# ml4ai/mliis

Measured on AMD Instinct MI355X. Metric: inner-loop images/sec (EfficientLab-6-3, 224x224, 5-shot), higher is better.
Workload: dtype f32 (the long-K decoder convs and their filter gradients with every operand split exactly into three bf16 terms on the matrix cores, 6 term products, f32 accumulate: fp32-equivalent products; everything else the fp32 instruction)

## Files before the change

### mliis_amd/csrc/conv_x3.hip

```cpp
#include "conv_gemm_kernels.hpp"

namespace mliis {

constexpr int kX3BM = 256;
#ifndef X3_PF
#define X3_PF 1
#endif
constexpr int kX3PF = X3_PF;

__global__ __launch_bounds__(128) void x3_pack_k(const float* __restrict__ theta, char* __restrict__ images, const long long* __restrict__ desc,
                                                  int ndesc) {
  x3_pack_block(theta, images, desc, ndesc, blockIdx.x, threadIdx.x);
}

struct X3Params {
  ConvGemmParams g;
  const char* image;
  int ncol16;
#ifdef X3_CLK
  unsigned long long* dbg;
#endif
};

template <int NT>
struct X3Sm {
  static constexpr int BN = 16 * NT;
  static constexpr int B_BYTES = NT * kX3Block;
  static constexpr int STAGES = 2;
  static constexpr int BYTES = STAGES * B_BYTES + 64;
};

template <int NT>
__device__ __forceinline__ void conv_x3_tile(const X3Params& q, char* __restrict__ sm, unsigned bx, int by, int it0, int it1,
                                             float* __restrict__ pdst) {
  constexpr int BN = 16 * NT;
  constexpr int B_BYTES = X3Sm<NT>::B_BYTES;
  constexpr int NB = (NT * 192 + 511) / 512;
  const ConvGemmParams& p = q.g;
  const int t = threadIdx.x, lane = t & 63;
  const int wave = __builtin_amdgcn_readfirstlane(t >> 6);
  const int l15 = lane & 15, g = lane >> 4;
  const long long M = (long long)p.Nimg * p.H * p.W;
  const long long m0 = (long long)bx * kX3BM;
  const int n0 = by * BN;
  const __amdgpu_buffer_rsrc_t rA = __builtin_amdgcn_make_buffer_rsrc((void*)p.A, 0, kBufRecords, 0x00020000);
  const __amdgpu_buffer_rsrc_t rB = __builtin_amdgcn_make_buffer_rsrc((void*)q.image, 0, kBufRecords, 0x00020000);

  const int wrow = wave * 32;
  unsigned a_row[2], a_taps[2];
#pragma unroll
  for (int rb = 0; rb < 2; ++rb) {
    const long long m = m0 + wrow + rb * 16 + l15;
    a_taps[rb] = 0;
    a_row[rb] = 0;
    if (m < M) {
      a_row[rb] = (unsigned)(m * p.lda * 4);
      if (p.ntaps > 1) {
        const int HWp = p.H * p.W;
        const int n = (int)(m / HWp);
        const int rem = (int)(m - (long long)n * HWp);
        const int h = rem / p.W, w_ = rem - h * p.W;
#pragma unroll
        for (int tp = 0; tp < 9; ++tp) {
          const int dh = (tp / 3 - 1) * p.dil * p.sign, dw = (tp % 3 - 1) * p.dil * p.sign;
          if ((unsigned)(h + dh) < (unsigned)p.H && (unsigned)(w_ + dw) < (unsigned)p.W) a_taps[rb] |= 1u << tp;
        }
      } else {
        a_taps[rb] = 1u;
      }
    }
  }
  int l_tap[2], l_c[2];
#pragma unroll
  for (int qd = 0; qd < 2; ++qd) {
    const int k0 = it0 * 32 + qd * 16 + g * 4;
    l_tap[qd] = k0 / p.C;
    l_c[qd] = k0 - l_tap[qd] * p.C;
  }
  int s_aleft = it1 - it0, s_bleft = it1 - it0;
  int ncol_here = q.ncol16 - by * NT;
  if (ncol_here > NT) ncol_here = NT;
  const unsigned b_lim = (unsigned)ncol_here * 192u;
  const unsigned b_step = (unsigned)q.ncol16 * kX3Block;
  unsigned b_voff[NB];
#pragma unroll
  for (int i = 0; i < NB; ++i) b_voff[i] = ((unsigned)t + 512u * i < b_lim) ? (unsigned)(by * NT) * kX3Block + ((unsigned)t + 512u * i) * 16u : kOob;
  unsigned s_boff = (unsigned)it0 * b_step;

  float4 ra[2][2];
  float4 ra2[2][2];
  u32x4 rbv[NB];
  const int tap_scale = p.dil * p.sign;
  auto load_a_into = [&](float4 (&ra)[2][2]) {
    const int adv = s_aleft > 1 ? 1 : 0;
    s_aleft -= adv;
#pragma unroll
    for (int qd = 0; qd < 2; ++qd) {
      const int tap = l_tap[qd];
      const int th = p.ntaps > 1 ? (tap * 11) >> 5 : 1, tw = p.ntaps > 1 ? tap - 3 * th : 1;
      const int dh = (th - 1) * tap_scale, dw = (tw - 1) * tap_scale;
      const unsigned koff = (unsigned)(((dh * p.W + dw) * p.lda + l_c[qd]) * 4);
      const unsigned tapbit = tap < p.ntaps ? 1u << tap : 0u;
#pragma unroll
      for (int rb = 0; rb < 2; ++rb) ra[rb][qd] = buf_ld4(rA, (a_taps[rb] & tapbit) != 0 ? a_row[rb] + koff : kOob);
      const int c_next = l_c[qd] + 32;
      const int wrap = c_next >= p.C ? 1 : 0;
      l_c[qd] = adv ? (wrap ? c_next - p.C : c_next) : l_c[qd];
      l_tap[qd] += adv & wrap;
    }
  };
  auto load_b_into = [&](u32x4 (&rbv)[NB]) {
#pragma unroll
    for (int i = 0; i < NB; ++i) {
      rbv[i] = __builtin_amdgcn_raw_buffer_load_b128(rB, (int)b_voff[i], (int)s_boff, 0);
    }
    const int adv = s_bleft > 1 ? 1 : 0;
    s_bleft -= adv;
    s_boff += adv ? b_step : 0u;
  };
  auto store_b_from = [&](char* buf, const u32x4 (&rbv)[NB]) {
#pragma unroll
    for (int i = 0; i < NB; ++i) {
      const int idx = t + 512 * i;
      char* d = (512 * (i + 1) <= NT * 192 || idx < NT * 192) ? buf + idx * 16 : sm + X3Sm<NT>::STAGES * B_BYTES + (t & 3) * 16;
      *reinterpret_cast<u32x4*>(d) = rbv[i];
    }
  };
  auto load_b = [&]() { load_b_into(rbv); };
  auto store_b = [&](char* buf) { store_b_from(buf, rbv); };
  bf16x8 a3[3][2], a3n[3][2];
  auto split_into = [&](const float4 (&ra)[2][2], bf16x8 (&a3)[3][2]) {
#pragma unroll
    for (int rb = 0; rb < 2; ++rb) {
      uint2 h0, m0_, l0, h1, m1, l1;
      split3(ra[rb][0], h0, m0_, l0);
      split3(ra[rb][1], h1, m1, l1);
      a3[0][rb] = __builtin_bit_cast(bf16x8, (u32x4){h0.x, h0.y, h1.x, h1.y});
      a3[1][rb] = __builtin_bit_cast(bf16x8, (u32x4){m0_.x, m0_.y, m1.x, m1.y});
      a3[2][rb] = __builtin_bit_cast(bf16x8, (u32x4){l0.x, l0.y, l1.x, l1.y});
    }
  };
  f32x4 acc[2][NT];
#pragma unroll
  for (int rb = 0; rb < 2; ++rb)
#pragma unroll
    for (int j = 0; j < NT; ++j) acc[rb][j] = (f32x4){0.f, 0.f, 0.f, 0.f};
  auto compute_split = [&](const char* buf, const float4 (&rs)[2][2]) {
    const char* pb = buf + g * 256 + l15 * 16;
    constexpr int PF = kX3PF;
    bf16x8 b3[PF + 1][3];
    uint2 sh[2][2], sm_[2][2], sl[2][2];
#pragma unroll
    for (int d = 0; d < PF; ++d)
      if (d < NT) {
#pragma unroll
        for (int pl = 0; pl < 3; ++pl) b3[d][pl] = *reinterpret_cast<const bf16x8*>(pb + d * kX3Block + pl * 1024);
      }
#pragma unroll
    for (int jn = 0; jn < NT; ++jn) {
#if defined(X3_ABL) && (X3_ABL & 2)
      if (jn + PF < NT && jn + PF < 2) {
#else
      if (jn + PF < NT) {
#endif
#pragma unroll
        for (int pl = 0; pl < 3; ++pl) b3[(jn + PF) % (PF + 1)][pl] = *reinterpret_cast<const bf16x8*>(pb + (jn + PF) * kX3Block + pl * 1024);
      }
#define X3_MM(PA, PB)                                                                                                           \
  acc[0][jn] = __builtin_amdgcn_mfma_f32_16x16x32_bf16(a3[PA][0], b3[jn % (PF + 1)][PB], acc[0][jn], 0, 0, 0);                \
  acc[1][jn] = __builtin_amdgcn_mfma_f32_16x16x32_bf16(a3[PA][1], b3[jn % (PF + 1)][PB], acc[1][jn], 0, 0, 0);
#if defined(X3_ABL) && (X3_ABL & 1)
      X3_MM(0, 0)
#else
      X3_MM(2, 0) X3_MM(0, 2) X3_MM(1, 1) X3_MM(1, 0) X3_MM(0, 1) X3_MM(0, 0)
#endif
#undef X3_MM
#pragma unroll
      for (int k = 0; k < 4; ++k)
        if ((k * NT) / 4 == jn) {
          uint2& h = sh[k >> 1][k & 1];
          uint2& m = sm_[k >> 1][k & 1];
          uint2& l = sl[k >> 1][k & 1];
#ifdef X3_NOSPLIT
          h = make_uint2(__float_as_uint(rs[k >> 1][k & 1].x), __float_as_uint(rs[k >> 1][k & 1].y));
          m = make_uint2(__float_as_uint(rs[k >> 1][k & 1].z), __float_as_uint(rs[k >> 1][k & 1].w));
          l = h;
#else
          split3(rs[k >> 1][k & 1], h, m, l);
#endif
          asm volatile("" : "+v"(h.x), "+v"(h.y), "+v"(m.x), "+v"(m.y), "+v"(l.x), "+v"(l.y));
        }
      __builtin_amdgcn_sched_barrier(0);
    }
#pragma unroll
    for (int rb = 0; rb < 2; ++rb) {
      a3n[0][rb] = __builtin_bit_cast(bf16x8, (u32x4){sh[rb][0].x, sh[rb][0].y, sh[rb][1].x, sh[rb][1].y});
      a3n[1][rb] = __builtin_bit_cast(bf16x8, (u32x4){sm_[rb][0].x, sm_[rb][0].y, sm_[rb][1].x, sm_[rb][1].y});
      a3n[2][rb] = __builtin_bit_cast(bf16x8, (u32x4){sl[rb][0].x, sl[rb][0].y, sl[rb][1].x, sl[rb][1].y});
    }
  };
#ifdef X3_CLK
  const unsigned long long ck0 = __builtin_amdgcn_s_memtime(), cr0 = __builtin_amdgcn_s_memrealtime();
  unsigned long long c_comp = 0, c_skel = 0, c_bar = 0, c_t = ck0;
#define X3_TICK(acc_) do { const unsigned long long n_ = __builtin_amdgcn_s_memtime(); acc_ += n_ - c_t; c_t = n_; } while (0)
#else
#define X3_TICK(acc_) do { } while (0)
#endif
  const int nper = it1 - it0;
  load_a_into(ra);
  load_b();
  store_b(sm);
  load_b();
  split_into(ra, a3);
  load_a_into(ra);
  load_a_into(ra2);
  lds_barrier();
  auto chunk = [&](char* cur, char* nxt, float4 (&rs)[2][2]) {
    compute_split(cur, rs);
    X3_TICK(c_comp);
#if !(defined(X3_ABL) && (X3_ABL & 8))
    store_b(nxt);
    load_b();
#endif
#if !(defined(X3_ABL) && (X3_ABL & 4))
    load_a_into(rs);
#endif
    X3_TICK(c_skel);
    lds_barrier();
    X3_TICK(c_bar);
#pragma unroll
    for (int pl = 0; pl < 3; ++pl)
#pragma unroll
      for (int rb = 0; rb < 2; ++rb) a3[pl][rb] = a3n[pl][rb];
  };
  {
    int it = 0;
    for (; it + 2 <= nper; it += 2) {
      chunk(sm, sm + B_BYTES, ra);
      chunk(sm + B_BYTES, sm, ra2);
    }
    if (it < nper) chunk(sm, sm + B_BYTES, ra);
  }
#ifndef X3_NO_DRAIN
  asm volatile("s_waitcnt vmcnt(0)" ::: "memory");
#endif
#ifdef X3_CLK
  if (q.dbg != nullptr && lane == 0 && (wave & 3) == 0) {
    unsigned long long* d = q.dbg + ((long long)blockIdx.x * 2 + (wave >> 2)) * 8;
    if (d[0] == 0) {
      d[0] = ck0;
      d[1] = cr0;
      d[2] = __builtin_amdgcn_s_memtime();
      d[3] = __builtin_amdgcn_s_memrealtime();
      d[4] = c_comp;
      d[5] = c_skel;
      d[6] = c_bar;
      d[7] = nper;
    }
  }
#endif
#pragma unroll
  for (int rb = 0; rb < 2; ++rb)
#pragma unroll
    for (int r = 0; r < 4; ++r) {
      const int row = wrow + rb * 16 + g * 4 + r;
      if (m0 + row >= M) continue;
#pragma unroll
      for (int j = 0; j < NT; ++j)
        if (n0 + j * 16 + l15 < p.Nout) pdst[(long long)row * BN + j * 16 + l15] = acc[rb][j][r];
    }
}

template <int NT>
__global__ __launch_bounds__(512) void conv_x3_k(X3Params q, SkPlan k) {
  __shared__ __attribute__((aligned(16))) char sm[X3Sm<NT>::BYTES];
  constexpr int BN = 16 * NT;
#ifndef X3_NO_CLAIM
  asm volatile("v_mov_b32 v255, 0" ::: "v255");
#endif
#ifndef X3_NO_XCD
  const int part = (int)xcd_remap(blockIdx.x, gridDim.x);
#else
  const int part = blockIdx.x;
#endif
  int lo = part * k.ipp;
  const int total = k.rem * k.nchunks;
  int hi = lo + k.ipp;
  if (hi > total) hi = total;
#pragma unroll 1
  while (lo < hi) {
    const int rt = lo / k.nchunks, c0 = lo - rt * k.nchunks;
    int c1 = c0 + (hi - lo);
    if (c1 > k.nchunks) c1 = k.nchunks;
    const int first = (rt * k.nchunks) / k.ipp;
    float* dst = k.slab + ((long long)rt * k.smax + (part - first)) * (kX3BM * BN);
    conv_x3_tile<NT>(q, sm, rt / k.gy, rt % k.gy, c0, c1, dst);
    lo += c1 - c0;
    __syncthreads();
  }
}

constexpr int kX3Fix = 4;
template <int NT>
__global__ __launch_bounds__(1024) void x3_fixup_k(ConvGemmParams p, SkPlan k) {
  constexpr int BN = 16 * NT, QN = BN / 4;
  constexpr int QS = QN <= 32 ? 32 : 64;
  constexpr int RL = 1024 / QS;
  constexpr int RPT = kX3BM / kX3Fix / RL;
  __shared__ float4 red[2][RL][QS];
  const int t = threadIdx.x, q = t % QS, rl = t / QS;
  const int rt = blockIdx.x, sub = blockIdx.y;
  const unsigned tau = k.full + rt;
  const int bx = tau / k.gy, by = tau % k.gy;
  const long long M = (long long)p.Nimg * p.H * p.W;
  const int r0 = sub * (kX3BM / kX3Fix);
  const long long m0 = (long long)bx * kX3BM + r0;
  const int n = by * BN + q * 4;
  const bool cok = q < QN && n < p.Nout;
  const int first = (rt * k.nchunks) / k.ipp;
  int last = ((rt + 1) * k.nchunks - 1) / k.ipp;
  if (last > k.parts - 1) last = k.parts - 1;
  const int nslots = last - first + 1;
  const float* base = k.slab + ((long long)rt * k.smax * kX3BM + r0) * BN + q * 4;
  float4 s1 = f4zero(), s2 = f4zero();
  if (cok) {
    const float4 bv = p.bias != nullptr ? ld4(p.bias + n) : f4zero();
    const long long HWp = (long long)p.H * p.W;
    float4 v[RPT];
#pragma unroll
    for (int i = 0; i < RPT; ++i) v[i] = (m0 + rl + RL * i < M) ? ld4(base + (long long)(rl + RL * i) * BN) : f4zero();
    for (int z = 1; z < nslots; ++z) {
      float4 u[RPT];
#pragma unroll
      for (int i = 0; i < RPT; ++i) u[i] = (m0 + rl + RL * i < M) ? ld4(base + ((long long)z * kX3BM + rl + RL * i) * BN) : f4zero();
#pragma unroll
      for (int i = 0; i < RPT; ++i) v[i] = f4add(v[i], u[i]);
    }
#pragma unroll
    for (int i = 0; i < RPT; ++i) {
      const long long m = m0 + rl + RL * i;
      if (m >= M) continue;
      float4 o = f4add(v[i], bv);
      if (p.border_bias != nullptr) {
        const int ni = (int)(m / HWp);
        const int rem = (int)(m - (long long)ni * HWp);
        const int h = rem / p.W, w_ = rem - h * p.W;
        const int cls = (h == 0 ? 0 : (h == p.H - 1 ? 2 : 1)) * 3 + (w_ == 0 ? 0 : (w_ == p.W - 1 ? 2 : 1));
        o = f4add(o, ld4(p.border_bias + ((long long)ni * 9 + cls) * p.Nout + n));
      }
      float* dst = p.Cmat + m * p.ldc + n;
      if (p.accumulate) o = f4add(o, ld4(dst));
      st4(dst, o);
      if (p.stats_swish) o = make_float4(swish_f(o.x), swish_f(o.y), swish_f(o.z), swish_f(o.w));
      s1 = f4add(s1, o);
      s2 = f4fma(o, o, s2);
    }
  }
  if (p.stats_part == nullptr) return;
  red[0][rl][q] = s1;
  red[1][rl][q] = s2;
  __syncthreads();
  if (t < 2 * QS) {
    const int v = t / QS, qq = t % QS;
    const int nn = by * BN + qq * 4;
    if (qq < QN && nn < p.Nout) {
      float4 a = red[v][0][qq];
#pragma unroll 8
      for (int r = 1; r < RL; ++r) a = f4add(a, red[v][r][qq]);
      st4(p.stats_part + (((long long)bx * kX3Fix + sub) * 2 + v) * p.Nout + nn, a);
    }
  }
}

typedef short x3_v4s __attribute__((ext_vector_type(4)));
__device__ __forceinline__ uint2 ds_read_tr16(const char* p) {
  const x3_v4s r = __builtin_amdgcn_ds_read_tr16_b64_v4i16((x3_v4s __attribute__((address_space(3)))*)(p));
  return __builtin_bit_cast(uint2, r);
}
constexpr int kF3Rows = 32;
constexpr int kF3Plane = kF3Rows * 256;
constexpr int kF3Stage = 6 * kF3Plane;
__device__ __forceinline__ int f3_swz(int row) { return (row & 3) | (((row >> 3) & 1) << 2); }

template <int BCI>
struct F3Sm {
  static constexpr int XQ = BCI / 4;
  static constexpr int XP = BCI * 2;
  static constexpr int X_PLANE = kF3Rows * XP;
  static constexpr int STAGE = 3 * X_PLANE + 3 * kF3Plane;
};
template <int NT, int BCI>
__device__ __forceinline__ void conv_filter_x3_body(const FilterGradParams& p, char* __restrict__ sm, int bx, int by, int bz) {
  constexpr int BN = 16 * NT;
  constexpr bool WIDE = BCI == 256;
  constexpr int XQ = F3Sm<BCI>::XQ, XP = F3Sm<BCI>::XP, X_PLANE = F3Sm<BCI>::X_PLANE, STAGE = F3Sm<BCI>::STAGE;
  constexpr int X_PER_THREAD = kF3Rows * XQ / 512;
  constexpr int X_ROWS_PASS = 512 / XQ;
  constexpr int D_TOTAL = kF3Rows * (BN / 4);
  constexpr int D_PER_THREAD = (D_TOTAL + 511) / 512;
  constexpr int NT0 = WIDE ? NT : (NT + 1) / 2, NT1 = WIDE ? 0 : NT / 2;
  const int t = threadIdx.x, lane = t & 63;
  const int wave = __builtin_amdgcn_readfirstlane(t >> 6);
  const int cib = WIDE ? wave : (wave & 3), half = WIDE ? 0 : (wave >> 2);
  const int l15 = lane & 15, g = lane >> 4;
  const int M = p.Nimg * p.H * p.W;
  const bool mt = p.multitap != 0;
  const int cblocks = mt ? 1 : (p.C + BCI - 1) / BCI;
  const int tap = mt ? 0 : bx / cblocks;
  const int ci0 = mt ? 0 : (bx - tap * cblocks) * BCI;
  const int n0 = by * BN;
#ifdef F3_SAMEBZ
  const int mbeg = 0;
#else
  const int mbeg = bz * p.rows_per_split;
#endif
  int mend = mbeg + p.rows_per_split;
  if (mend > M) mend = M;
  const int HW = p.H * p.W;
  const int adv_h = kF3Rows / p.W, adv_w = kF3Rows - adv_h * p.W;
  const __amdgpu_buffer_rsrc_t rX = __builtin_amdgcn_make_buffer_rsrc((void*)p.X, 0, kBufRecords, 0x00020000);
  const __amdgpu_buffer_rsrc_t rD = __builtin_amdgcn_make_buffer_rsrc((void*)p.dY, 0, kBufRecords, 0x00020000);

  const int x_cq = t % XQ, x_r0 = t / XQ;
  int l_tap = tap, l_c = ci0 + x_cq * 4;
  if (mt) {
    l_tap = (x_cq * 4) / p.C;
    l_c = x_cq * 4 - l_tap * p.C;
  }
  const bool x_cok = mt ? l_tap < p.ntaps : l_c < p.C;
  int dh = 0, dw = 0;
  if (p.ntaps > 1) {
    dh = (l_tap / 3 - 1) * p.dil;
    dw = (l_tap % 3 - 1) * p.dil;
  }
  int x_m[X_PER_THREAD], x_h[X_PER_THREAD], x_w[X_PER_THREAD];
  unsigned x_off[X_PER_THREAD];
#pragma unroll
  for (int i = 0; i < X_PER_THREAD; ++i) {
    const int m = mbeg + x_r0 + X_ROWS_PASS * i;
    x_m[i] = m;
    const int n = m / HW;
    const int rem = m - n * HW;
    x_h[i] = rem / p.W;
    x_w[i] = rem - x_h[i] * p.W;
    x_off[i] = (unsigned)((((long long)m + (long long)dh * p.W + dw) * p.ldx + l_c) * 4);
  }
  const unsigned x_step = (unsigned)(kF3Rows * p.ldx * 4);
  int d_m[D_PER_THREAD];
  unsigned d_off[D_PER_THREAD];
  bool d_ok[D_PER_THREAD];
  int d_lds[D_PER_THREAD];
#pragma unroll
  for (int i = 0; i < D_PER_THREAD; ++i) {
    const int idx = t + 512 * i;
    const int r = idx / (BN / 4), nq = idx - r * (BN / 4);
    d_m[i] = mbeg + r;
    d_ok[i] = (idx < D_TOTAL) && (n0 + nq * 4 < p.Nout);
    d_off[i] = (unsigned)((((long long)mbeg + r) * p.lddy + n0 + nq * 4) * 4);
    d_lds[i] = idx < D_TOTAL ? 3 * X_PLANE + r * 256 + (((nq >> 2) ^ f3_swz(r)) * 32) + (nq & 3) * 8 : -1;
  }
  const unsigned d_step = (unsigned)(kF3Rows * p.lddy * 4);
  int x_lds[X_PER_THREAD];
#pragma unroll
  for (int i = 0; i < X_PER_THREAD; ++i) {
    const int r = x_r0 + X_ROWS_PASS * i;
    const int ch = x_cq >> 2;
    x_lds[i] = r * XP + (((ch & ~7) | ((ch & 7) ^ f3_swz(r))) * 32) + (x_cq & 3) * 8;
  }

  float4 rxa[X_PER_THREAD], rda[D_PER_THREAD], rxb[X_PER_THREAD], rdb[D_PER_THREAD];
  auto load_chunk = [&](float4 (&rx)[X_PER_THREAD], float4 (&rd)[D_PER_THREAD]) {
#pragma unroll
    for (int i = 0; i < X_PER_THREAD; ++i) {
      const bool ok = x_cok & (x_m[i] < mend) & ((unsigned)(x_h[i] + dh) < (unsigned)p.H) & ((unsigned)(x_w[i] + dw) < (unsigned)p.W);
      rx[i] = buf_ld4(rX, ok ? x_off[i] : kOob);
      x_m[i] += kF3Rows;
      x_off[i] += x_step;
      x_w[i] += adv_w;
      x_h[i] += adv_h;
      if (x_w[i] >= p.W) {
        x_w[i] -= p.W;
        ++x_h[i];
      }
      if (x_h[i] >= p.H) x_h[i] -= (x_h[i] / p.H) * p.H;
    }
#pragma unroll
    for (int i = 0; i < D_PER_THREAD; ++i) {
      rd[i] = buf_ld4(rD, (d_ok[i] & (d_m[i] < mend)) ? d_off[i] : kOob);
      d_m[i] += kF3Rows;
      d_off[i] += d_step;
    }
  };
  constexpr int NP = X_PER_THREAD + D_PER_THREAD;
  uint2 th[NP], tm[NP], tl[NP];
  auto split_piece = [&](int k, const float4 (&rx)[X_PER_THREAD], const float4 (&rd)[D_PER_THREAD]) {
#ifdef F3_NOSPLIT
    {
      const float4 v_ = k < X_PER_THREAD ? rx[k < X_PER_THREAD ? k : 0] : rd[k >= X_PER_THREAD ? k - X_PER_THREAD : 0];
      th[k] = make_uint2(__float_as_uint(v_.x), __float_as_uint(v_.y));
      tm[k] = make_uint2(__float_as_uint(v_.z), __float_as_uint(v_.w));
      tl[k] = th[k];
    }
#else
    split3(k < X_PER_THREAD ? rx[k < X_PER_THREAD ? k : 0] : rd[k >= X_PER_THREAD ? k - X_PER_THREAD : 0], th[k], tm[k], tl[k]);
#endif
    asm volatile("" : "+v"(th[k].x), "+v"(th[k].y), "+v"(tm[k].x), "+v"(tm[k].y), "+v"(tl[k].x), "+v"(tl[k].y));
  };
  auto store_terms = [&](char* buf) {
#pragma unroll
    for (int i = 0; i < X_PER_THREAD; ++i) {
      char* d = buf + x_lds[i];
      *reinterpret_cast<uint2*>(d) = th[i];
      *reinterpret_cast<uint2*>(d + X_PLANE) = tm[i];
      *reinterpret_cast<uint2*>(d + 2 * X_PLANE) = tl[i];
    }
#pragma unroll
    for (int i = 0; i < D_PER_THREAD; ++i) {
      if (512 * (i + 1) <= D_TOTAL || d_lds[i] >= 0) {
        char* d = buf + d_lds[i];
        *reinterpret_cast<uint2*>(d) = th[X_PER_THREAD + i];
        *reinterpret_cast<uint2*>(d + kF3Plane) = tm[X_PER_THREAD + i];
        *reinterpret_cast<uint2*>(d + 2 * kF3Plane) = tl[X_PER_THREAD + i];
      }
    }
  };
  constexpr int NTW = NT0;
  f32x4 acc[2][NTW];
#pragma unroll
  for (int i = 0; i < 2; ++i)
#pragma unroll
    for (int j = 0; j < NTW; ++j) acc[i][j] = (f32x4){0.f, 0.f, 0.f, 0.f};
  const int fq = l15 >> 2, fp = l15 & 3;
  int a_row[2], d_row[2], a_sw[2];
#pragma unroll
  for (int hh = 0; hh < 2; ++hh) {
    const int r = 8 * g + 4 * hh + fq;
    a_row[hh] = r * XP + fp * 8;
    d_row[hh] = r * 256 + fp * 8;
    a_sw[hh] = f3_swz(r);
  }
  const bool wave_live = mt ? cib * 32 < p.ntaps * p.C : ci0 + cib * 32 < p.C;
  const int jn0 = half == 0 ? 0 : NT0;
  const int njn = half == 0 ? NT0 : NT1;
  auto frag = [&](const char* plane, const int (&row)[2], int chunk16) {
    const uint2 lo = ds_read_tr16(plane + row[0] + (((chunk16 & ~7) | ((chunk16 & 7) ^ a_sw[0])) * 32));
    const uint2 hi = ds_read_tr16(plane + row[1] + (((chunk16 & ~7) | ((chunk16 & 7) ^ a_sw[1])) * 32));
    return __builtin_bit_cast(bf16x8, (u32x4){lo.x, lo.y, hi.x, hi.y});
  };
  auto compute_split = [&](const char* buf, const float4 (&rx)[X_PER_THREAD], const float4 (&rd)[D_PER_THREAD]) {
    bf16x8 a3[3][2], b3[2][3];
    if (wave_live) {
#pragma unroll
      for (int pl = 0; pl < 3; ++pl)
#pragma unroll
        for (int rb = 0; rb < 2; ++rb) a3[pl][rb] = frag(buf + pl * X_PLANE, a_row, cib * 2 + rb);
#pragma unroll
      for (int pl = 0; pl < 3; ++pl) b3[0][pl] = frag(buf + 3 * X_PLANE + pl * kF3Plane, d_row, jn0);
    }
#pragma unroll
    for (int j = 0; j < NTW; ++j) {
      if (wave_live && j < njn) {
        if (j + 1 < NTW && j + 1 < njn) {
#pragma unroll
          for (int pl = 0; pl < 3; ++pl) b3[(j + 1) & 1][pl] = frag(buf + 3 * X_PLANE + pl * kF3Plane, d_row, jn0 + j + 1);
        }
#define X3_MM(PA, PB)                                                                                            \
  acc[0][j] = __builtin_amdgcn_mfma_f32_16x16x32_bf16(a3[PA][0], b3[j & 1][PB], acc[0][j], 0, 0, 0);           \
  acc[1][j] = __builtin_amdgcn_mfma_f32_16x16x32_bf16(a3[PA][1], b3[j & 1][PB], acc[1][j], 0, 0, 0);
#ifdef F3_NOMFMA
        X3_MM(0, 0)
#else
        X3_MM(2, 0) X3_MM(0, 2) X3_MM(1, 1) X3_MM(1, 0) X3_MM(0, 1) X3_MM(0, 0)
#endif
#undef X3_MM
      }
#ifndef F3_NOSTAGE
#pragma unroll
      for (int k = 0; k < NP; ++k)
        if ((k * NTW) / NP == j) split_piece(k, rx, rd);
#endif
      __builtin_amdgcn_sched_barrier(0);
    }
  };

  const int nchunks = (mend - mbeg + kF3Rows - 1) / kF3Rows;
  load_chunk(rxa, rda);
#pragma unroll
  for (int k = 0; k < NP; ++k) split_piece(k, rxa, rda);
  store_terms(sm);
  load_chunk(rxa, rda);
  load_chunk(rxb, rdb);
  lds_barrier();
  auto trip = [&](char* cur, char* nxt, float4 (&rx)[X_PER_THREAD], float4 (&rd)[D_PER_THREAD]) {
    compute_split(cur, rx, rd);
#ifndef F3_NOSTAGE
    store_terms(nxt);
#endif
    load_chunk(rx, rd);
    lds_barrier();
  };
  int it = 0;
  for (; it + 2 <= nchunks; it += 2) {
    trip(sm, sm + STAGE, rxa, rda);
    trip(sm + STAGE, sm, rxb, rdb);
  }
  if (it < nchunks) trip(sm, sm + STAGE, rxa, rda);
#ifndef X3_NO_DRAIN
  asm volatile("s_waitcnt vmcnt(0)" ::: "memory");
#endif

  const long long Ktot = (long long)p.ntaps * p.C;
#pragma unroll
  for (int rb = 0; rb < 2; ++rb)
#pragma unroll
    for (int r = 0; r < 4; ++r) {
      const int ci = ci0 + cib * 32 + rb * 16 + g * 4 + r;
      if (ci >= (mt ? p.ntaps * p.C : p.C)) continue;
#pragma unroll
      for (int j = 0; j < NTW; ++j) {
        const int n = n0 + (jn0 + j) * 16 + l15;
        if (j < njn && n < p.Nout) p.partial[((long long)bz * Ktot + (long long)tap * p.C + ci) * p.Nout + n] = acc[rb][j][r];
      }
    }
}

template <int NT>
__global__ __launch_bounds__(512) void conv_filter_x3_batched_k(const long long* __restrict__ desc, int nprob, int tile_ci) {
  __shared__ __attribute__((aligned(16))) char sm[2 * F3Sm<256>::STAGE];
#ifndef F3_NO_CLAIM
  asm volatile("v_mov_b32 v255, 0" ::: "v255");
#endif
  const int b = blockIdx.x;
  int j = 0;
  for (int k = 1; k < nprob; ++k)
    if (b >= (int)desc[k * kFilterDescWords + 15]) j = k;
  const long long* d = desc + (long long)j * kFilterDescWords;
  const int ks = (int)(d[11] & 0xff);
  const FilterGradParams p{reinterpret_cast<const float*>(d[0]), (int)d[4], (int)d[6], (int)d[7], (int)d[8], (int)d[9], ks * ks, (int)d[12],
                           reinterpret_cast<const float*>(d[1]), (int)d[5], (int)d[10], reinterpret_cast<float*>(d[3]),
                           (int)(d[13] & 0xffffffffLL), nullptr, (int)(d[13] >> 32), 0, 0};
  const int gx = (int)(d[14] & 0xfffff), gy = (int)((d[14] >> 20) & 0xfffff);
  const int local = b - (int)d[15];
  const int bx = local % gx, r = local / gx;
  if (tile_ci == 256 && p.multitap == 0 && p.C > 128) conv_filter_x3_body<NT, 256>(p, sm, bx, r % gy, r / gy);
  else conv_filter_x3_body<NT, 128>(p, sm, bx, r % gy, r / gy);
}

bool launch_filter_batched_x3(int nt, const long long* desc, int nprob, int blocks, int tile_ci, hipStream_t stream) {
  dim3 grid(blocks), block(512);
#define L(NT_) hipLaunchKernelGGL((conv_filter_x3_batched_k<NT_>), grid, block, 0, stream, desc, nprob, tile_ci); return true;
  switch (nt) {
    case 4: L(4)
    case 5: L(5)
    case 6: L(6)
    case 7: L(7)
    case 8: L(8)
    default: return false;
  }
#undef L
}

struct X3Plan {
  int nt, gx, gy, nchunks;
  int full, rem, parts, ipp, smax;
  size_t slab_floats() const { return (size_t)rem * smax * kX3BM * (16 * nt); }
};
constexpr int kX3MinPart = 4;

#ifndef X3_MAX_NT
#define X3_MAX_NT 9
#endif
static int x3_pick_nt(int Nout) {
  int best = 1;
  double best_cost = 1e30;
  const int tiles = (Nout + 15) / 16;
  for (int nt = 1; nt <= X3_MAX_NT; ++nt) {
    const int blocks = (tiles + nt - 1) / nt;
    const double cost = (double)(blocks * nt * 16) / (double)Nout * (1.0 + 0.08 * (8 - nt));
    if (cost < best_cost - 1e-9 || (cost < best_cost + 1e-9 && nt > best)) {
      best_cost = cost;
      best = nt;
    }
  }
  return best;
}

static inline int x3_chunks(int ntaps, int Cred) { return (ntaps * Cred + 31) / 32; }
static X3Plan x3_plan(long long M, int Nout, int ntaps, int Cred, int num_cus) {
  X3Plan g;
  g.nt = x3_pick_nt(Nout);
  g.gy = (Nout + g.nt * 16 - 1) / (g.nt * 16);
  g.gx = (int)((M + kX3BM - 1) / kX3BM);
  g.nchunks = x3_chunks(ntaps, Cred);
  const int slots = num_cus;
  while (g.nt > 2 && (long long)g.gx * g.gy * g.nchunks < (long long)slots * 2 * kX3MinPart) {
    g.nt = (g.nt + 1) / 2;
    g.gy = (Nout + g.nt * 16 - 1) / (g.nt * 16);
  }
  const long long tiles = (long long)g.gx * g.gy;
  g.full = 0;
  g.rem = (int)tiles;
  const long long total = tiles * g.nchunks;
  long long parts = slots;
  if (parts > 8LL * tiles) parts = 8LL * tiles;
  if (total / parts < kX3MinPart) parts = total / kX3MinPart;
  if (parts < 1) parts = 1;
  g.ipp = (int)((total + parts - 1) / parts);
  g.parts = (int)((total + g.ipp - 1) / g.ipp);
  g.smax = (g.nchunks + g.ipp - 1) / g.ipp + 1;
  return g;
}

static int g_x3_cus = 0;
static int x3_num_cus() {
  if (g_x3_cus == 0) {
    int dev = 0;
    hipDeviceProp_t prop;
    g_x3_cus = (hipGetDevice(&dev) == hipSuccess && hipGetDeviceProperties(&prop, dev) == hipSuccess && prop.multiProcessorCount > 0)
                   ? prop.multiProcessorCount
                   : 256;
  }
  return g_x3_cus;
}

static void x3_launch(const X3Plan& g, const X3Params& q_, float* slab, hipStream_t stream) {
  X3Params q = q_;
#ifdef X3_CLK
  q.dbg = getenv("MLIIS_X3_STAMPS") ? (unsigned long long*)strtoull(getenv("MLIIS_X3_STAMPS"), nullptr, 0) : nullptr;
#endif
  const SkPlan k{g.full, g.rem, g.parts, g.ipp, g.nchunks, g.smax, g.gy, slab};
  dim3 grid(g.parts), block(512);
#define L(NT_)                                                                                  \
  hipLaunchKernelGGL((conv_x3_k<NT_>), grid, block, 0, stream, q, k);                           \
  hipLaunchKernelGGL((x3_fixup_k<NT_>), dim3(g.rem, kX3Fix), dim3(1024), 0, stream, q.g, k);    \
  break;
  switch (g.nt) {
    case 1: L(1)
    case 2: L(2)
    case 3: L(3)
    case 4: L(4)
    case 5: L(5)
    case 6: L(6)
    case 7: L(7)
    case 8: L(8)
    default: L(9)
  }
#undef L
}

static int x3_shape_check(const char* name, int Nimg, int H, int W, int Cred, int Nout, int ksize, int dil) {
  MLIIS_REQUIRE(Nimg > 0 && H > 0 && W > 0 && Cred >= 32 && Nout > 0, MLIIS_ERR_ARG, "%s: bad shape (the reduced channel count must be >= 32)", name);
  MLIIS_REQUIRE((Cred & 3) == 0 && (Nout & 3) == 0, MLIIS_ERR_ARG, "%s: channel counts must be multiples of 4", name);
  MLIIS_REQUIRE(ksize == 1 || ksize == 3, MLIIS_ERR_UNSUPPORTED, "%s: kernel size %d unsupported (1 or 3)", name, ksize);
  MLIIS_REQUIRE(dil >= 1, MLIIS_ERR_ARG, "%s: dilation must be >= 1", name);
  return MLIIS_OK;
}

}

using namespace mliis;

extern "C" {

size_t mliis_x3_image_bytes(int Cred, int Nout, int ksize) {
  return (size_t)x3_chunks(ksize * ksize, Cred) * ((Nout + 15) / 16) * kX3Block;
}

int mliis_x3_image_blocks(int Cred, int Nout, int ksize) { return x3_chunks(ksize * ksize, Cred) * ((Nout + 15) / 16); }

int mliis_x3_pack_weights(const float* theta, void* images, const long long* desc, int ndesc, int total_blocks, hipStream_t stream) {
  MLIIS_REQUIRE(theta && images && desc && ndesc >= 1 && ndesc <= 64 && total_blocks >= 1, MLIIS_ERR_ARG, "x3_pack_weights: bad arguments");
  MLIIS_REQUIRE(aligned16(theta) && aligned16(images) && aligned16(desc), MLIIS_ERR_ALIGN, "x3_pack_weights: pointers must be 16-byte aligned");
  hipLaunchKernelGGL(x3_pack_k, dim3(total_blocks), dim3(128), 0, stream, theta, reinterpret_cast<char*>(images), desc, ndesc);
  MLIIS_CHECK_LAUNCH("x3_pack_weights");
  return MLIIS_OK;
}

size_t mliis_conv2d_x3_workspace_floats(int Nimg, int H, int W, int Cred, int Nout, int ksize) {
  return x3_plan((long long)Nimg * H * W, Nout, ksize * ksize, Cred, x3_num_cus()).slab_floats();
}

int mliis_conv2d_x3_plan(int Nimg, int H, int W, int Cred, int Nout, int ksize, int* plan) {
  MLIIS_REQUIRE(plan, MLIIS_ERR_ARG, "conv2d_x3_plan: null pointer");
  const X3Plan g = x3_plan((long long)Nimg * H * W, Nout, ksize * ksize, Cred, x3_num_cus());
  plan[0] = g.nt; plan[1] = g.gx; plan[2] = g.gy; plan[3] = g.full; plan[4] = g.parts; plan[5] = g.ipp;
  return MLIIS_OK;
}

int mliis_conv2d_fwd_x3(const float* x, int ldx, const void* image, size_t image_bytes, const float* bias, const float* border_bias, float* y, int ldy, int Nimg,
                        int H, int W, int Cin, int Cout, int ksize, int dil, int accumulate, float* stats_part, int stats_swish,
                        int* stats_nblk, float* ws, size_t ws_floats, hipStream_t stream) {
  int rc = x3_shape_check("conv2d_fwd_x3", Nimg, H, W, Cin, Cout, ksize, dil);
  if (rc) return rc;
  MLIIS_REQUIRE(x && image && y, MLIIS_ERR_ARG, "conv2d_fwd_x3: null pointer");
  MLIIS_REQUIRE(image_bytes == mliis_x3_image_bytes(Cin, Cout, ksize), MLIIS_ERR_ARG,
                "conv2d_fwd_x3: the weight image has %zu bytes, a forward image over %d reduced channels x %d columns (k = %d) has %zu -- packed for another "
                "window or direction?", image_bytes, Cin, Cout, ksize, mliis_x3_image_bytes(Cin, Cout, ksize));
  MLIIS_REQUIRE((ldx & 3) == 0 && ldx >= Cin && (ldy & 3) == 0 && ldy >= Cout, MLIIS_ERR_ARG, "conv2d_fwd_x3: bad leading dimensions");
  MLIIS_REQUIRE(aligned16(x) && aligned16(image) && aligned16(bias) && aligned16(y) && aligned16(border_bias) && aligned16(ws), MLIIS_ERR_ALIGN,
                "conv2d_fwd_x3: pointers must be 16-byte aligned");
  const long long M = (long long)Nimg * H * W;
  MLIIS_REQUIRE(M * ldx * 4 < (1LL << 31) && mliis_x3_image_bytes(Cin, Cout, ksize) < (1ULL << 31), MLIIS_ERR_UNSUPPORTED,
                "conv2d_fwd_x3: operand larger than 2 GiB (32-bit buffer offsets)");
  MLIIS_REQUIRE(border_bias == nullptr || (ksize == 3 && dil == 1 && H >= 2 && W >= 2), MLIIS_ERR_ARG,
                "conv2d_fwd_x3: border_bias needs a 3x3 dilation-1 conv on a map of at least 2x2");
  MLIIS_REQUIRE(stats_part == nullptr || (!accumulate && stats_nblk), MLIIS_ERR_ARG,
                "conv2d_fwd_x3: fused statistics need accumulate == 0 and a stats_nblk output");
  const X3Plan g = x3_plan(M, Cout, ksize * ksize, Cin, x3_num_cus());
  MLIIS_REQUIRE(g.slab_floats() == 0 || (ws != nullptr && g.slab_floats() <= ws_floats), MLIIS_ERR_WORKSPACE,
                "conv2d_fwd_x3: workspace too small (%zu needed, %zu given)", g.slab_floats(), ws_floats);
  X3Params q{};
  q.g = ConvGemmParams{x, ldx, Nimg, H, W, Cin, ksize * ksize, dil, +1, nullptr, 0, 0, Cout, y, ldy, bias, accumulate, nullptr, 0,
                       stats_part, stats_swish, nullptr, border_bias, 1.0f, nullptr};
  q.image = reinterpret_cast<const char*>(image);
  q.ncol16 = (Cout + 15) / 16;
  x3_launch(g, q, ws, stream);
  MLIIS_CHECK_LAUNCH("conv2d_fwd_x3");
  if (stats_nblk) *stats_nblk = stats_part != nullptr ? g.gx * kX3Fix : 0;
  return MLIIS_OK;
}

int mliis_conv2d_bwd_data_x3(const float* dy, int lddy, const void* image, size_t image_bytes, float* dx, int lddx, int Nimg, int H, int W, int Cin_out, int Cout,
                             int ksize, int dil, int accumulate, float* ws, size_t ws_floats, hipStream_t stream) {
  int rc = x3_shape_check("conv2d_bwd_data_x3", Nimg, H, W, Cout, Cin_out, ksize, dil);
  if (rc) return rc;
  MLIIS_REQUIRE(dy && image && dx, MLIIS_ERR_ARG, "conv2d_bwd_data_x3: null pointer");
  MLIIS_REQUIRE(image_bytes == mliis_x3_image_bytes(Cout, Cin_out, ksize), MLIIS_ERR_ARG,
                "conv2d_bwd_data_x3: the weight image has %zu bytes, a backward-data image over %d reduced channels x %d columns (k = %d) has %zu -- packed "
                "for another window or direction?", image_bytes, Cout, Cin_out, ksize, mliis_x3_image_bytes(Cout, Cin_out, ksize));
  MLIIS_REQUIRE((lddy & 3) == 0 && lddy >= Cout && (lddx & 3) == 0 && lddx >= Cin_out, MLIIS_ERR_ARG, "conv2d_bwd_data_x3: bad leading dimensions");
  MLIIS_REQUIRE(aligned16(dy) && aligned16(image) && aligned16(dx) && aligned16(ws), MLIIS_ERR_ALIGN,
                "conv2d_bwd_data_x3: pointers must be 16-byte aligned");
  const long long M = (long long)Nimg * H * W;
  MLIIS_REQUIRE(M * lddy * 4 < (1LL << 31) && mliis_x3_image_bytes(Cout, Cin_out, ksize) < (1ULL << 31), MLIIS_ERR_UNSUPPORTED,
                "conv2d_bwd_data_x3: operand larger than 2 GiB (32-bit buffer offsets)");
  const X3Plan g = x3_plan(M, Cin_out, ksize * ksize, Cout, x3_num_cus());
  MLIIS_REQUIRE(g.slab_floats() == 0 || (ws != nullptr && g.slab_floats() <= ws_floats), MLIIS_ERR_WORKSPACE,
                "conv2d_bwd_data_x3: workspace too small (%zu needed, %zu given)", g.slab_floats(), ws_floats);
  X3Params q{};
  q.g = ConvGemmParams{dy, lddy, Nimg, H, W, Cout, ksize * ksize, dil, -1, nullptr, 0, 0, Cin_out, dx, lddx, nullptr, accumulate, nullptr, 0,
                       nullptr, 0, nullptr, nullptr, 1.0f, nullptr};
  q.image = reinterpret_cast<const char*>(image);
  q.ncol16 = (Cin_out + 15) / 16;
  x3_launch(g, q, ws, stream);
  MLIIS_CHECK_LAUNCH("conv2d_bwd_data_x3");
  return MLIIS_OK;
}
}
```

Baseline: 3582.

## Interleave B stage/load and A prefetch into the MFMA loop, strength-reduce tap offsets

Moves the LDS store of the next B tile, the next global B load and the next A prefetch from after the compute loop into its middle and end, so their issue overlaps with matrix-core work instead of sitting between compute and the barrier. It also replaces the per-iteration tap/channel to offset computation (divides, multiplies) with incrementally updated byte offsets and tap bits, using precomputed column/row wrap deltas. The trade-off is higher register pressure inside the compute loop, plus an LDS write during reads of the other buffer. The offset update also assumes a channel wrap advances by exactly one tap, which holds only while the channel step does not exceed C.

```diff
diff --git a/mliis_amd/csrc/conv_x3.hip b/mliis_amd/csrc/conv_x3.hip
--- a/mliis_amd/csrc/conv_x3.hip
+++ b/mliis_amd/csrc/conv_x3.hip
@@ -70,12 +70,19 @@
       }
     }
   }
-  int l_tap[2], l_c[2];
+  const int tap_scale = p.dil * p.sign;
+  const unsigned t_col = (p.ntaps > 1 ? (unsigned)(tap_scale * p.lda * 4) : 0u) - 4u * (unsigned)p.C;
+  const unsigned t_row = (p.ntaps > 1 ? (unsigned)((p.W - 2) * tap_scale * p.lda * 4) : 0u) - 4u * (unsigned)p.C;
+  int l_c[2];
+  unsigned l_bit[2], l_off[2];
 #pragma unroll
   for (int qd = 0; qd < 2; ++qd) {
     const int k0 = it0 * 32 + qd * 16 + g * 4;
-    l_tap[qd] = k0 / p.C;
-    l_c[qd] = k0 - l_tap[qd] * p.C;
+    const int tap = k0 / p.C;
+    const int th = p.ntaps > 1 ? tap / 3 : 1, tw = p.ntaps > 1 ? tap - 3 * th : 1;
+    l_c[qd] = k0 - tap * p.C;
+    l_bit[qd] = 1u << tap;
+    l_off[qd] = (unsigned)((((th - 1) * p.W + (tw - 1)) * tap_scale * p.lda + l_c[qd]) * 4);
   }
   int s_aleft = it1 - it0, s_bleft = it1 - it0;
   int ncol_here = q.ncol16 - by * NT;
@@ -90,23 +97,19 @@
   float4 ra[2][2];
   float4 ra2[2][2];
   u32x4 rbv[NB];
-  const int tap_scale = p.dil * p.sign;
   auto load_a_into = [&](float4 (&ra)[2][2]) {
-    const int adv = s_aleft > 1 ? 1 : 0;
-    s_aleft -= adv;
+    const int adv = s_aleft > 1 ? 32 : 0;
+    s_aleft -= adv ? 1 : 0;
 #pragma unroll
     for (int qd = 0; qd < 2; ++qd) {
-      const int tap = l_tap[qd];
-      const int th = p.ntaps > 1 ? (tap * 11) >> 5 : 1, tw = p.ntaps > 1 ? tap - 3 * th : 1;
-      const int dh = (th - 1) * tap_scale, dw = (tw - 1) * tap_scale;
-      const unsigned koff = (unsigned)(((dh * p.W + dw) * p.lda + l_c[qd]) * 4);
-      const unsigned tapbit = tap < p.ntaps ? 1u << tap : 0u;
-#pragma unroll
-      for (int rb = 0; rb < 2; ++rb) ra[rb][qd] = buf_ld4(rA, (a_taps[rb] & tapbit) != 0 ? a_row[rb] + koff : kOob);
-      const int c_next = l_c[qd] + 32;
-      const int wrap = c_next >= p.C ? 1 : 0;
-      l_c[qd] = adv ? (wrap ? c_next - p.C : c_next) : l_c[qd];
-      l_tap[qd] += adv & wrap;
+      const unsigned bit = l_bit[qd], off = l_off[qd];
+#pragma unroll
+      for (int rb = 0; rb < 2; ++rb) ra[rb][qd] = buf_ld4(rA, (a_taps[rb] & bit) != 0 ? a_row[rb] + off : kOob);
+      const int c_next = l_c[qd] + adv;
+      const bool wrap = c_next >= p.C;
+      l_c[qd] = wrap ? c_next - p.C : c_next;
+      l_off[qd] = off + 4u * (unsigned)adv + (wrap ? ((bit & 0x124u) != 0 ? t_row : t_col) : 0u);
+      l_bit[qd] = wrap ? bit << 1 : bit;
     }
   };
   auto load_b_into = [&](u32x4 (&rbv)[NB]) {
@@ -145,7 +148,7 @@
   for (int rb = 0; rb < 2; ++rb)
 #pragma unroll
     for (int j = 0; j < NT; ++j) acc[rb][j] = (f32x4){0.f, 0.f, 0.f, 0.f};
-  auto compute_split = [&](const char* buf, const float4 (&rs)[2][2]) {
+  auto compute_split = [&](const char* buf, float4 (&rs)[2][2], char* nxt) {
     const char* pb = buf + g * 256 + l15 * 16;
     constexpr int PF = kX3PF;
     bf16x8 b3[PF + 1][3];
@@ -190,6 +193,15 @@
 #endif
           asm volatile("" : "+v"(h.x), "+v"(h.y), "+v"(m.x), "+v"(m.y), "+v"(l.x), "+v"(l.y));
         }
+#if !(defined(X3_ABL) && (X3_ABL & 8))
+      if (jn == NT / 2) {
+        store_b(nxt);
+        load_b();
+      }
+#endif
+#if !(defined(X3_ABL) && (X3_ABL & 4))
+      if (jn == NT - 1) load_a_into(rs);
+#endif
       __builtin_amdgcn_sched_barrier(0);
     }
 #pragma unroll
@@ -216,15 +228,8 @@
   load_a_into(ra2);
   lds_barrier();
   auto chunk = [&](char* cur, char* nxt, float4 (&rs)[2][2]) {
-    compute_split(cur, rs);
+    compute_split(cur, rs, nxt);
     X3_TICK(c_comp);
-#if !(defined(X3_ABL) && (X3_ABL & 8))
-    store_b(nxt);
-    load_b();
-#endif
-#if !(defined(X3_ABL) && (X3_ABL & 4))
-    load_a_into(rs);
-#endif
     X3_TICK(c_skel);
     lds_barrier();
     X3_TICK(c_bar);
```

After: 3580, median of 6. No clear change (-0.1%).
